# Crocodoctopus/zkstark

Measured on AMD Instinct MI355X. Metric: field-elements/s through LDE+Merkle+FRI (full STARK-101 prover), higher is better.
Workload: dtype u32 (mod 3*2^30+1) + SHA-256

## Files before the change

### zkstark_amd/csrc/kernels.hip

```cpp
#include "kernels.hpp"

#include <cstdlib>

#include "field.hpp"
#include "fieldhash_f64.hpp"
#include "sha256_quad.hpp"
#include "sha256.hpp"

namespace zk {

__device__ __forceinline__ uint32_t pow_lookup(const PowTable& t, uint32_t e) {
    return mont_mul(t.hi[e >> t.lo_bits], t.lo[e & ((1u << t.lo_bits) - 1u)]);
}

constexpr uint32_t R2_MONT = R2;

__device__ uint32_t mont_inv(uint32_t a) {
    uint32_t r = R1, b = a;
    uint32_t e = P - 2;
#pragma unroll 1
    for (int i = 0; i < 32; ++i) {
        if (e & 1) r = mont_mul(r, b);
        b = mont_mul(b, b);
        e >>= 1;
// ... 316 lines not shown
            f2[k] = B == 1 ? fw[k + 2] : fw[k + 4];
            inv2[k] = B == 1 ? iw[k + 2] : iw[k + 4];
            zz[k] = B == 1 ? a.zz[0] : a.zz[k & 1];
        }
    }
    uint32_t x = mont_mul(pow_lookup(a.htab, (uint32_t)i), a.w_mont);
    const uint32_t h = pow_lookup(a.htab, 1u);
    uint32_t r[4];
#pragma unroll
    for (int k = 0; k < 4; ++k) {
        r[k] = compose_eval<false>(a, f0[k], f1[k], f2[k], inv0[k], inv2[k], x, zz[k], a.first, a.last, a.alpha0_mont, a.alpha1g2_mont, 0u);
        if (k < 3) x = mont_mul(x, h);
    }
    reinterpret_cast<uint4*>(a.cp)[i >> 2] = make_uint4(r[0], r[1], r[2], r[3]);
}

hipError_t launch_compose(const ComposeArgs& a, hipStream_t s, Profiler* prof) {
    size_t N = (size_t)1 << a.logN;
    ScopedKernelTimer tm(prof, K_COMPOSE, 8.0 * (double)N, s);
    const bool aligned = ((reinterpret_cast<uintptr_t>(a.f) | reinterpret_cast<uintptr_t>(a.inv_xm1) | reinterpret_cast<uintptr_t>(a.cp)) & 15u) == 0;
    if (a.logN >= 4 && aligned) {
        uint32_t blocks = (uint32_t)((N / 4 + 255) / 256);
        hipLaunchKernelGGL(compose_kernel4, dim3(blocks), dim3(256), 0, s, a);
    } else {
        uint32_t blocks = (uint32_t)((N + 255) / 256);
        hipLaunchKernelGGL(compose_kernel, dim3(blocks), dim3(256), 0, s, a);
    }
    return hipGetLastError();
}

struct FoldRaw { uint32_t u, v, x_hi, x_lo; };
__device__ __forceinline__ FoldRaw fold_fetch(const FoldArgs& a, size_t i) {
    const size_t half = (size_t)1 << (a.log_m - 1);
    const uint32_t e = (uint32_t)(i << a.round);
    FoldRaw r;
    r.u = a.in[i]; r.v = a.in[i + half];
    r.x_hi = a.hinv.hi[e >> a.hinv.lo_bits]; r.x_lo = a.hinv.lo[e & ((1u << a.hinv.lo_bits) - 1u)];
    return r;
}
__device__ __forceinline__ uint32_t fold_finish(const FoldArgs& a, const FoldRaw& r) {
    uint32_t xinv = mont_mul(r.x_hi, r.x_lo);
    uint32_t s = mont_mul(add(r.u, r.v), a.inv2_mont);
    uint32_t d = mont_mul(mont_mul(sub(r.u, r.v), xinv), a.c_mont);
    return add(s, d);
}
__device__ __forceinline__ uint32_t fold_at(const FoldArgs& a, size_t i) { return fold_finish(a, fold_fetch(a, i)); }

__global__ __launch_bounds__(256) void fri_fold_kernel(FoldArgs a) {
    size_t i = (size_t)blockIdx.x * blockDim.x + threadIdx.x;
    if (i >= ((size_t)1 << (a.log_m - 1))) return;
    a.out[i] = fold_at(a, i);
}

__global__ __launch_bounds__(256) void fri_fold_kernel4(FoldArgs a) {
    const size_t half = (size_t)1 << (a.log_m - 1);
    const size_t i = ((size_t)blockIdx.x * blockDim.x + threadIdx.x) * 4;
    if (i >= half) return;
    const uint4 u = reinterpret_cast<const uint4*>(a.in)[i >> 2], v = reinterpret_cast<const uint4*>(a.in)[(i + half) >> 2];
    const uint32_t uu[4] = {u.x, u.y, u.z, u.w}, vv[4] = {v.x, v.y, v.z, v.w};
    uint32_t xinv = pow_lookup(a.hinv, (uint32_t)(i << a.round));
    const uint32_t step = pow_lookup(a.hinv, 1u << a.round);
    uint32_t r[4];
#pragma unroll
    for (int k = 0; k < 4; ++k) {
        const uint32_t sm = mont_mul(add(uu[k], vv[k]), a.inv2_mont);
        const uint32_t d = mont_mul(mont_mul(sub(uu[k], vv[k]), xinv), a.c_mont);
        r[k] = add(sm, d);
        if (k < 3) xinv = mont_mul(xinv, step);
    }
    reinterpret_cast<uint4*>(a.out)[i >> 2] = make_uint4(r[0], r[1], r[2], r[3]);
}

hipError_t launch_fri_fold(const FoldArgs& a, hipStream_t s, Profiler* prof) {
    size_t half = (size_t)1 << (a.log_m - 1);
    ScopedKernelTimer tm(prof, K_FOLD, 12.0 * (double)half, s);
    const bool aligned = ((reinterpret_cast<uintptr_t>(a.in) | reinterpret_cast<uintptr_t>(a.out)) & 15u) == 0;
    if (half >= 4 && aligned) {
        uint32_t blocks = (uint32_t)((half / 4 + 255) / 256);
        hipLaunchKernelGGL(fri_fold_kernel4, dim3(blocks), dim3(256), 0, s, a);
    } else {
        uint32_t blocks = (uint32_t)((half + 255) / 256);
        hipLaunchKernelGGL(fri_fold_kernel, dim3(blocks), dim3(256), 0, s, a);
    }
    return hipGetLastError();
}


__constant__ FieldHashConsts g_fh_consts;
__constant__ FieldHashConsts64 g_fh_consts64;

template <int HASH> struct Hasher;
template <> struct Hasher<0> {
    static __device__ __forceinline__ Digest leaf(uint32_t v) { return sha256_leaf(v); }
    static __device__ __forceinline__ Digest inner(const Digest& l, const Digest& r) { return sha256_inner(l, r); }
};
template <> struct Hasher<1> {
    static __device__ __forceinline__ Digest leaf(uint32_t v) { return fieldhash_leaf64(v, g_fh_consts64); }
    static __device__ __forceinline__ Digest inner(const Digest& l, const Digest& r) { return fieldhash_inner64(l, r, g_fh_consts64); }
};

struct PlainSrc {
    const uint32_t* vals;
    using Raw = uint32_t;
    __device__ __forceinline__ Raw fetch(size_t pos) const { return vals[pos]; }
    __device__ __forceinline__ uint32_t finish(const Raw& r, size_t) const { return r; }
    __device__ __forceinline__ uint32_t load(size_t pos) const { return vals[pos]; }
};
struct FoldSrc {
    FoldArgs a;
    using Raw = FoldRaw;
    __device__ __forceinline__ void prepare() { if (a.dyn) a.c_mont = *a.dyn; }
    __device__ __forceinline__ Raw fetch(size_t pos) const { return fold_fetch(a, pos); }
    __device__ __forceinline__ uint32_t finish(const Raw& r, size_t pos) const { uint32_t v = fold_finish(a, r); a.out[pos] = v; return v; }
    __device__ __forceinline__ uint32_t load(size_t pos) const { return finish(fetch(pos), pos); }
};
struct ComposeSrc {
    ComposeArgs a;
    using Raw = size_t;
    __device__ __forceinline__ Raw fetch(size_t pos) const { return pos; }
    __device__ __forceinline__ uint32_t finish(const Raw& r, size_t) const { return load(r); }
    __device__ __forceinline__ uint32_t load(size_t pos) const { uint32_t v = compose_at(a, pos); a.cp[pos] = v; return v; }
};

struct ComposeBlockSrc {
    ComposeBlockArgs b;
    using Raw = size_t;
    __device__ __forceinline__ uint32_t f_at(size_t t) const {
        const uint32_t gmask = (1u << b.lg) - 1u;
        if (t >> b.log_m) {
            const size_t v = t - ((size_t)1 << b.log_m);
            return b.halo[(v & gmask) * b.halo_stride + (v >> b.lg)];
        }
        const uint32_t log_cl = b.lg + b.log_cnt;
        const size_t piece = ((t >> log_cl) << b.lg) | (t & gmask);
        return b.a.f[(piece << b.log_cnt) | ((t & (((size_t)1 << log_cl) - 1)) >> b.lg)];
    }
    __device__ __forceinline__ Raw fetch(size_t pos) const { return pos; }
    __device__ __forceinline__ uint32_t finish(const Raw& r, size_t) const { return load(r); }
    __device__ __forceinline__ uint32_t load(size_t pos) const {
        const ComposeArgs& a = b.a;
        const size_t B = (size_t)1 << a.log_b;
        const uint32_t f0 = f_at(pos), f1 = f_at(pos + B), f2 = f_at(pos + 2 * B);
        const uint32_t x = mont_mul(pow_lookup(a.htab, b.e0 + (uint32_t)pos), a.w_mont);
        return compose_eval<false>(a, f0, f1, f2, a.inv_xm1[pos], a.inv_xm1[pos + 2 * B], x, a.zz[pos & (B - 1)], a.first, a.last, a.alpha0_mont,
                                   a.alpha1g2_mont, 0u);
    }
};

struct ComposeBatchSrc {
    ComposeArgs a;
    const BatchChal* chal;
    using Raw = size_t;
    __device__ __forceinline__ Raw fetch(size_t pos) const { return pos; }
    __device__ __forceinline__ uint32_t finish(const Raw& r, size_t) const { return load(r); }
    __device__ __forceinline__ uint32_t load(size_t pos) const {
        const size_t b = pos >> a.logN, i = pos & (((size_t)1 << a.logN) - 1);
        const BatchChal c = chal[b];
        uint32_t v = compose_core<true>(a, a.f + (b << a.logN), c.first, c.last, c.alpha0_mont, c.alpha1g2_mont, c.alpha2_mont, i);
        a.cp[pos] = v;
        return v;
    }
};
struct FoldBatchSrc {
    FoldArgs a;
    const BatchChal* chal;
    using Raw = size_t;
    __device__ __forceinline__ Raw fetch(size_t pos) const { return pos; }
    __device__ __forceinline__ uint32_t finish(const Raw& r, size_t) const { return load(r); }
    __device__ __forceinline__ uint32_t load(size_t pos) const {
        const uint32_t lh = a.log_m - 1;
        const size_t half = (size_t)1 << lh, b = pos >> lh, i = pos & (half - 1);
        const uint32_t* in = a.in + (b << a.log_m);
        uint32_t u = in[i], v = in[i + half];
        uint32_t xinv = pow_lookup(a.hinv, (uint32_t)(i << a.round));
        uint32_t s = mont_mul(add(u, v), a.inv2_mont);
        uint32_t d = mont_mul(mont_mul(sub(u, v), xinv), chal[b].c_mont);
        uint32_t r = add(s, d);
        a.out[pos] = r;
        return r;
    }
};

struct InterleaveSrc {
    const uint32_t* recv;
    uint32_t log_parts, log_cnt;
    using Raw = uint32_t;
    __device__ __forceinline__ uint32_t load(size_t pos) const {
        return recv[((pos & (((size_t)1 << log_parts) - 1)) << log_cnt) | (pos >> log_parts)];
    }
    __device__ __forceinline__ Raw fetch(size_t pos) const { return load(pos); }
    __device__ __forceinline__ uint32_t finish(const Raw& r, size_t) const { return r; }
};

template <class S> __device__ __forceinline__ auto src_prepare(S& s, int) -> decltype(s.prepare(), void()) { s.prepare(); }
template <class S> __device__ __forceinline__ void src_prepare(S&, long) {}

constexpr int kMerkleThreads = 256;
constexpr uint32_t kMerkleMaxK = 4;

__device__ __forceinline__ void store_digest(uint32_t* nodes, size_t node, const Digest& d) {
    uint4* q = reinterpret_cast<uint4*>(nodes + node * 8);
    q[0] = make_uint4(d.w[0], d.w[1], d.w[2], d.w[3]);
    q[1] = make_uint4(d.w[4], d.w[5], d.w[6], d.w[7]);
}
__device__ __forceinline__ Digest load_digest(const uint32_t* nodes, size_t node) {
    const uint4* q = reinterpret_cast<const uint4*>(nodes + node * 8);
    uint4 lo = q[0], hi = q[1];
    Digest d;
    d.w[0] = lo.x; d.w[1] = lo.y; d.w[2] = lo.z; d.w[3] = lo.w;
    d.w[4] = hi.x; d.w[5] = hi.y; d.w[6] = hi.z; d.w[7] = hi.w;
    return d;
}

__device__ __forceinline__ Digest lds_digest(const uint4* p) {
    uint4 lo = p[0], hi = p[1];
    Digest d;
    d.w[0] = lo.x; d.w[1] = lo.y; d.w[2] = lo.z; d.w[3] = lo.w;
    d.w[4] = hi.x; d.w[5] = hi.y; d.w[6] = hi.z; d.w[7] = hi.w;
    return d;
}

template <class SRC, bool LEAF, int HASH>
__global__ __launch_bounds__(kMerkleThreads) void merkle_subtree_kernel(SRC src, uint32_t* nodes,
                                                                        uint32_t depth_in, uint32_t k, size_t off) {
    extern __shared__ __attribute__((aligned(16))) uint4 stage[];
    src_prepare(src, 0);
    const uint32_t lane = threadIdx.x & 63u, wave = threadIdx.x >> 6;
    const size_t gwave = (size_t)blockIdx.x * (kMerkleThreads / 64) + wave;
    const size_t base = (gwave << (6 + k)) + off;
    const size_t in_base = ((size_t)1 << depth_in) - 1;
    uint4* my = stage + (size_t)wave * (k + 1) * 128;
    uint4* scratch = my + (size_t)k * 128;
    typename SRC::Raw raw;
    Digest dnext;
    uint32_t val = 0;
    if (LEAF) val = src.load(base + lane - off);
    else dnext = load_digest(nodes, in_base + base + lane);
#pragma unroll 1
    for (uint32_t i = 0; i < (1u << k); ++i) {
        Digest d;
        const size_t pos = base + (size_t)i * 64 + lane;
        const bool more = i + 1 < (1u << k);
        if (LEAF) {
            if (more) raw = src.fetch(pos + 64 - off);
            d = Hasher<HASH>::leaf(val);
            store_digest(nodes, in_base + pos, d);
        } else {
            d = dnext;
            if (more) dnext = load_digest(nodes, in_base + pos + 64);
        }
        uint32_t idx = i, lvl = 0;
#pragma unroll 1
        while (lvl < k) {
            uint4* left = my + lvl * 128;
            uint4* grp = (idx & 1u) ? scratch : left;
            grp[2 * lane] = make_uint4(d.w[0], d.w[1], d.w[2], d.w[3]);
            grp[2 * lane + 1] = make_uint4(d.w[4], d.w[5], d.w[6], d.w[7]);
            if (!(idx & 1u)) break;
            __builtin_amdgcn_fence(__ATOMIC_RELEASE, "wavefront");
            __builtin_amdgcn_wave_barrier();
            const uint4* x = (lane < 32u ? left : scratch - 128) + 4 * lane;
            Digest l = lds_digest(x), r = lds_digest(x + 2);
            __builtin_amdgcn_wave_barrier();
            d = Hasher<HASH>::inner(l, r);
            idx >>= 1;
            ++lvl;
            store_digest(nodes, (((size_t)1 << (depth_in - lvl)) - 1) + (base >> lvl) + (size_t)idx * 64 + lane, d);
        }
        if (LEAF && more) val = src.finish(raw, pos + 64 - off);
    }
}

constexpr int kWgThreads = 256;
#ifndef ZK_FIELD_ROW_MAX_NODES
#define ZK_FIELD_ROW_MAX_NODES 16
#endif
constexpr uint32_t kFieldRowMaxNodes = ZK_FIELD_ROW_MAX_NODES;
static_assert(kFieldRowMaxNodes >= 16 && kFieldRowMaxNodes <= 64, "the row form takes at most four passes of 16 nodes");
#ifndef ZK_FIELD_QUAD_MAX_NODES
#define ZK_FIELD_QUAD_MAX_NODES 64
#endif
constexpr uint32_t kFieldQuadMaxNodes = ZK_FIELD_QUAD_MAX_NODES;
static_assert(kFieldQuadMaxNodes <= 128, "the quad form takes at most two passes of 64 nodes");
#ifndef ZK_FIELD_ROW_LEAF_MAX
#define ZK_FIELD_ROW_LEAF_MAX 32
#endif
constexpr uint32_t kFieldRowLeafMax = ZK_FIELD_ROW_LEAF_MAX;
static_assert(kFieldRowLeafMax <= 64, "the row form takes at most four passes of 16 leaves");
constexpr uint32_t kWgMaxLog = 10;

__device__ __forceinline__ void lds_store(uint4* p, const Digest& d) {
    p[0] = make_uint4(d.w[0], d.w[1], d.w[2], d.w[3]);
    p[1] = make_uint4(d.w[4], d.w[5], d.w[6], d.w[7]);
}

#ifndef ZK_WG_RELAXED_PUBLISH
#define ZK_WG_RELAXED_PUBLISH 1
#endif
constexpr bool kWgRelaxedPublish = ZK_WG_RELAXED_PUBLISH != 0;
__device__ __forceinline__ void publish_node(uint32_t* nodes, size_t node, const uint4* lvl0, uint32_t tid) {
    if (tid < 8) __hip_atomic_store(nodes + node * 8 + tid, reinterpret_cast<const uint32_t*>(lvl0)[tid], __ATOMIC_RELAXED, __HIP_MEMORY_SCOPE_AGENT);
    asm volatile("s_waitcnt vmcnt(0)" ::: "memory");
}
__device__ __forceinline__ Digest load_digest_agent(const uint32_t* nodes, size_t node) {
    const unsigned long long* q = reinterpret_cast<const unsigned long long*>(nodes + node * 8);
    Digest d;
#pragma unroll
    for (int i = 0; i < 4; ++i) {
        const unsigned long long v = __hip_atomic_load(q + i, __ATOMIC_RELAXED, __HIP_MEMORY_SCOPE_AGENT);
        d.w[2 * i] = (uint32_t)v; d.w[2 * i + 1] = (uint32_t)(v >> 32);
    }
    return d;
}

#ifdef ZK_WG_TRACE
constexpr uint32_t kWgTraceSlots = 48, kWgTraceLaunches = 8192;
__device__ unsigned long long g_wg_trace[kWgTraceLaunches][kWgTraceSlots];
__device__ unsigned int g_wg_trace_n, g_wg_trace_cur;
#define WG_STAMP(slot) do { if (threadIdx.x == 0 && wg_rec < kWgTraceLaunches && (slot) < kWgTraceSlots) g_wg_trace[wg_rec][(slot)] = __builtin_amdgcn_s_memrealtime(); } while (0)
#else
#define WG_STAMP(slot) do { } while (0)
#endif

template <class SRC, bool LEAF, int HASH>
__global__ __launch_bounds__(kWgThreads) void merkle_wg_kernel(SRC src, uint32_t* nodes, uint32_t depth_in, uint32_t j,
                                                               MailArgs mail, size_t off, uint32_t j2, uint32_t lds_log) {
    extern __shared__ __attribute__((aligned(16))) uint4 lvl[];
    src_prepare(src, 0);
    uint32_t* xch = reinterpret_cast<uint32_t*>(lvl + ((size_t)2 << lds_log));
    const uint32_t tid = threadIdx.x;
    uint32_t cnt = 1u << j;
    size_t first = ((size_t)blockIdx.x << j) + off;
    uint32_t d_in = depth_in, lv = j;
    const size_t in_base = ((size_t)1 << depth_in) - 1;
    QuadLane ql;
    if (HASH == 0) ql = quad_lane(tid);
#ifdef ZK_WG_TRACE
    uint32_t wg_rec = 0xffffffffu;
    if (blockIdx.x == 0 && tid == 0) {
        wg_rec = atomicAdd(&g_wg_trace_n, 1u);
        __hip_atomic_store(&g_wg_trace_cur, wg_rec, __ATOMIC_RELAXED, __HIP_MEMORY_SCOPE_AGENT);
        if (wg_rec < kWgTraceLaunches) {
            for (uint32_t i = 0; i < kWgTraceSlots; ++i) g_wg_trace[wg_rec][i] = 0;
            g_wg_trace[wg_rec][0] = (unsigned long long)depth_in | ((unsigned long long)j << 8) | ((unsigned long long)j2 << 16) | ((unsigned long long)(LEAF ? 1 : 0) << 24) |
                                    ((unsigned long long)HASH << 25) | ((unsigned long long)(mail.mailbox ? mail.top + 1 : 0) << 26) | ((unsigned long long)gridDim.x << 32);
        }
    }
    WG_STAMP(1);
#endif
    constexpr uint32_t kPer = (1u << kWgMaxLog) / kWgThreads;
    if (LEAF && HASH == 1 && cnt <= kFieldRowLeafMax) {
        const uint32_t g = tid & 15u, grp = tid >> 4;
#pragma unroll 1
        for (uint32_t b = 0; b * 16 < cnt; ++b) {
            const uint32_t i = b * 16 + grp;
            const uint32_t ii = i < cnt ? i : 0u;
            const uint32_t v = src.finish(src.fetch(first + ii - off), first + ii - off);
            const uint32_t word = g == 0 ? v : g == 15 ? 1u : 0u;
            const uint32_t res = fieldhash_inner_row16_f64(word, g, g_fh_consts64);
            if (i < cnt && g < 8) {
                nodes[(in_base + first + i) * 8 + g] = res;
                reinterpret_cast<uint32_t*>(&lvl[2 * i])[g] = res;
            }
        }
    } else if (LEAF) {
        typename SRC::Raw raw[kPer] = {};
#pragma unroll
        for (uint32_t u = 0; u < kPer; ++u)
            if (tid + u * kWgThreads < cnt) raw[u] = src.fetch(first + tid + u * kWgThreads - off);
#pragma unroll 1
        for (uint32_t i = tid; i < cnt; i += kWgThreads) {
            const Digest d = Hasher<HASH>::leaf(src.finish(raw[0], first + i - off));
            store_digest(nodes, in_base + first + i, d);
            lds_store(&lvl[2 * i], d);
#pragma unroll
            for (uint32_t u = 0; u + 1 < kPer; ++u) raw[u] = raw[u + 1];
        }
    } else {
        Digest dd[kPer];
#pragma unroll
        for (uint32_t u = 0; u < kPer; ++u)
            if (tid + u * kWgThreads < cnt) dd[u] = load_digest(nodes, in_base + first + tid + u * kWgThreads);
#pragma unroll
        for (uint32_t u = 0; u < kPer; ++u)
            if (tid + u * kWgThreads < cnt) lds_store(&lvl[2 * (tid + u * kWgThreads)], dd[u]);
    }
    if (LEAF && mail.dump_src) __threadfence();
    __syncthreads();
    WG_STAMP(2);
#pragma unroll 1
  for (uint32_t phase = 0;; ++phase) {
#pragma unroll 1
    for (uint32_t t = 1; t <= lv; ++t) {
        const uint32_t w = cnt >> t;
        const size_t out_base = (((size_t)1 << (d_in - t)) - 1) + (first >> t);
        WG_STAMP((phase ? 24u : 2u) + t - 1u);
        if (HASH == 0 && w <= 64) {
            const uint32_t lane = tid & 63u, wave = tid >> 6;
            const uint32_t node = wave * 16 + (lane >> 4) * 4 + (lane & 3u), role = (lane >> 2) & 3u;
            const bool busy = wave * 16 < w;
            uint32_t o[4];
            if (busy) sha256_inner_quad(reinterpret_cast<const uint32_t*>(&lvl[4 * (node < w ? node : 0u)]), ql, o);
            __syncthreads();
            if (busy && node < w && role < 2) {
                const uint4 v = make_uint4(o[0], o[1], o[2], o[3]);
                lvl[2 * node + (role ^ 1u)] = v;
                reinterpret_cast<uint4*>(nodes + (out_base + node) * 8)[role ^ 1u] = v;
            }
            __syncthreads();
            continue;
        }
        if (HASH == 0 && w <= 128) {
            const bool is_main = tid < 128;
            const uint32_t node = tid & 127u;
            const bool active = node < w;
            uint32_t wv[16];
            uint32_t st[8];
            if (active) {
                Digest l = lds_digest(&lvl[4 * node]), r = lds_digest(&lvl[4 * node + 2]);
#pragma unroll
                for (int i = 0; i < 8; ++i) { wv[i] = l.w[i]; wv[8 + i] = r.w[i]; st[i] = SHA_IV[i]; }
            }
            uint32_t* xb0 = xch;
            uint32_t* xb1 = xch + 16 * 128;
            if (active) {
                if (is_main) sha256_rounds16<0>(st, wv);
                else { sha256_schedule16(wv);
#pragma unroll
                       for (int i = 0; i < 16; ++i) xb0[i * 128 + node] = wv[i]; }
            }
            __syncthreads();
            if (active) {
                if (is_main) {
#pragma unroll
                    for (int i = 0; i < 16; ++i) wv[i] = xb0[i * 128 + node];
                    sha256_rounds16<16>(st, wv);
                } else { sha256_schedule16(wv);
#pragma unroll
                         for (int i = 0; i < 16; ++i) xb1[i * 128 + node] = wv[i]; }
            }
            __syncthreads();
            if (active) {
                if (is_main) {
#pragma unroll
                    for (int i = 0; i < 16; ++i) wv[i] = xb1[i * 128 + node];
                    sha256_rounds16<32>(st, wv);
                } else { sha256_schedule16(wv);
#pragma unroll
                         for (int i = 0; i < 16; ++i) xb0[i * 128 + node] = wv[i]; }
            }
            __syncthreads();
            Digest d0;
            if (active && is_main) {
#pragma unroll
                for (int i = 0; i < 16; ++i) wv[i] = xb0[i * 128 + node];
                sha256_rounds16<48>(st, wv);
#pragma unroll
                for (int i = 0; i < 8; ++i) d0.w[i] = st[i] + SHA_IV[i];
                uint32_t pad[16] = {0x80000000u, 0, 0, 0, 0, 0, 0, 0, 0, 0, 0, 0, 0, 0, 0, 512u};
                sha256_compress(d0.w, pad);
            }
            __syncthreads();
            if (active && is_main) { lds_store(&lvl[2 * node], d0); store_digest(nodes, out_base + node, d0); }
            __syncthreads();
            continue;
        }
        if (HASH == 1 && w > kFieldRowMaxNodes && w <= kFieldQuadMaxNodes) {
            const uint32_t q = tid & 3u, grp = tid >> 2;
            uint32_t res[2][4];
#pragma unroll
            for (uint32_t b = 0; b < 2; ++b) {
                if (b * 64 >= w) break;
                const uint32_t node = b * 64 + grp;
                const uint4 v = lvl[4 * (node < w ? node : 0u) + q];
                const uint32_t in[4] = {v.x, v.y, v.z, v.w};
                fieldhash_inner_quad_f64(in, q, res[b], g_fh_consts64);
            }
            __syncthreads();
#pragma unroll
            for (uint32_t b = 0; b < 2; ++b) {
                if (b * 64 >= w) break;
                const uint32_t node = b * 64 + grp;
                if (node < w && q < 2) {
                    const uint4 o = make_uint4(res[b][0], res[b][1], res[b][2], res[b][3]);
                    lvl[2 * node + q] = o;
                    reinterpret_cast<uint4*>(nodes + (out_base + node) * 8)[q] = o;
                }
            }
            __syncthreads();
            continue;
        }
        if (HASH == 1 && w <= kFieldRowMaxNodes) {
            const uint32_t g = tid & 15u, grp = tid >> 4;
            uint32_t res[4];
#pragma unroll
            for (uint32_t b = 0; b < 4; ++b) {
                if (b * 16 >= w) break;
                const uint32_t node = b * 16 + grp;
                const uint32_t* words = reinterpret_cast<const uint32_t*>(&lvl[4 * (node < w ? node : 0u)]);
                res[b] = fieldhash_inner_row16_f64(words[g], g, g_fh_consts64);
            }
            __syncthreads();
#pragma unroll
            for (uint32_t b = 0; b < 4; ++b) {
                if (b * 16 >= w) break;
                const uint32_t node = b * 16 + grp;
                if (node < w && g < 8) {
                    reinterpret_cast<uint32_t*>(&lvl[2 * node])[g] = res[b];
                    nodes[(out_base + node) * 8 + g] = res[b];
                }
            }
            __syncthreads();
            continue;
        }
        Digest d0, d1;
        const bool a0 = tid < w, a1 = tid + kWgThreads < w;
        if (a0) d0 = Hasher<HASH>::inner(lds_digest(&lvl[4 * tid]), lds_digest(&lvl[4 * tid + 2]));
        if (a1) d1 = Hasher<HASH>::inner(lds_digest(&lvl[4 * (tid + kWgThreads)]), lds_digest(&lvl[4 * (tid + kWgThreads) + 2]));
        __syncthreads();
        if (a0) { lds_store(&lvl[2 * tid], d0); store_digest(nodes, out_base + tid, d0); }
        if (a1) { lds_store(&lvl[2 * (tid + kWgThreads)], d1); store_digest(nodes, out_base + tid + kWgThreads, d1); }
        __syncthreads();
    }
    WG_STAMP((phase ? 24u : 2u) + lv);
    if (phase == 1 || j2 == 0) break;
    __shared__ uint32_t go_on;
    if (gridDim.x > 1) {
        if (kWgRelaxedPublish) {
            publish_node(nodes, (((size_t)1 << (depth_in - j)) - 1) + blockIdx.x, lvl, tid);
        } else {
            asm volatile("s_waitcnt vmcnt(0)" ::: "memory");
            __syncthreads();
        }
    }
    if (tid == 0) {
        uint32_t last = 1;
        if (gridDim.x > 1) {
            last = (kWgRelaxedPublish ? __hip_atomic_fetch_add(mail.counter + 1, 1u, __ATOMIC_RELAXED, __HIP_MEMORY_SCOPE_AGENT)
                                      : __hip_atomic_fetch_add(mail.counter + 1, 1u, __ATOMIC_ACQ_REL, __HIP_MEMORY_SCOPE_AGENT)) == gridDim.x - 1;
            if (last) __hip_atomic_store(mail.counter + 1, 0u, __ATOMIC_RELAXED, __HIP_MEMORY_SCOPE_AGENT);
        }
        go_on = last;
    }
    __syncthreads();
    if (!go_on) return;
    if (kWgRelaxedPublish && LEAF && mail.dump_src) __builtin_amdgcn_fence(__ATOMIC_ACQUIRE, "agent");
#ifdef ZK_WG_TRACE
    if (tid == 0) wg_rec = __hip_atomic_load(&g_wg_trace_cur, __ATOMIC_RELAXED, __HIP_MEMORY_SCOPE_AGENT);
    WG_STAMP(15);
#endif
    d_in = depth_in - j; lv = j2; cnt = gridDim.x; first = 0;
    {
        const size_t base2 = ((size_t)1 << d_in) - 1;
        Digest dd[kPer];
#pragma unroll
        for (uint32_t u = 0; u < kPer; ++u)
            if (tid + u * kWgThreads < cnt)
                dd[u] = (kWgRelaxedPublish && gridDim.x > 1) ? load_digest_agent(nodes, base2 + tid + u * kWgThreads) : load_digest(nodes, base2 + tid + u * kWgThreads);
#pragma unroll
        for (uint32_t u = 0; u < kPer; ++u)
            if (tid + u * kWgThreads < cnt) lds_store(&lvl[2 * (tid + u * kWgThreads)], dd[u]);
    }
    __syncthreads();
    WG_STAMP(16);
  }
    if (mail.mailbox && depth_in - j - j2 == mail.top && off == 0) {
        __shared__ uint32_t is_last;
        const bool relaxed = kWgRelaxedPublish && gridDim.x > 1 && j2 == 0 && mail.dump_src == nullptr;
        if (relaxed) publish_node(nodes, (((size_t)1 << mail.top) - 1) + blockIdx.x, lvl, tid);
        if (tid == 0) {
            uint32_t last = 1;
            if (gridDim.x > 1 && j2 == 0) {
                last = (relaxed ? __hip_atomic_fetch_add(mail.counter, 1u, __ATOMIC_RELAXED, __HIP_MEMORY_SCOPE_AGENT)
                                : __hip_atomic_fetch_add(mail.counter, 1u, __ATOMIC_ACQ_REL, __HIP_MEMORY_SCOPE_AGENT)) == gridDim.x - 1;
                if (last) __hip_atomic_store(mail.counter, 0u, __ATOMIC_RELAXED, __HIP_MEMORY_SCOPE_AGENT);
            }
            is_last = last;
        }
        __syncthreads();
        if (is_last) {
#ifdef ZK_WG_TRACE
            if (tid == 0 && wg_rec == 0xffffffffu) wg_rec = __hip_atomic_load(&g_wg_trace_cur, __ATOMIC_RELAXED, __HIP_MEMORY_SCOPE_AGENT);
            WG_STAMP(40);
#endif
            const uint4* sq = reinterpret_cast<const uint4*>(nodes + (((size_t)1 << mail.top) - 1) * 8);
            uint4* dq = reinterpret_cast<uint4*>(mail.mailbox + kMailDigests);
            if (relaxed) {
                for (uint32_t i = tid; i < (1u << mail.top); i += kWgThreads) {
                    const Digest d = load_digest_agent(nodes, (((size_t)1 << mail.top) - 1) + i);
                    dq[2 * i] = make_uint4(d.w[0], d.w[1], d.w[2], d.w[3]);
                    dq[2 * i + 1] = make_uint4(d.w[4], d.w[5], d.w[6], d.w[7]);
                }
            } else {
                for (uint32_t i = tid; i < (2u << mail.top); i += kWgThreads) dq[i] = sq[i];
            }
            if (mail.dump_src) {
                const uint4* sv = reinterpret_cast<const uint4*>(mail.dump_src);
                uint4* dv = reinterpret_cast<uint4*>(mail.mailbox + mail.vals_off);
                for (uint32_t i = tid; i < (1u << mail.dump_log) / 4; i += kWgThreads) dv[i] = sv[i];
            }
            __threadfence_system();
            __syncthreads();
            WG_STAMP(41);
            if (tid == 0) __hip_atomic_store(&mail.mailbox[0], mail.seq, __ATOMIC_RELEASE, __HIP_MEMORY_SCOPE_SYSTEM);
            WG_STAMP(42);
        }
    }
}

#ifdef ZK_WG_TRACE
void dump_wg_trace() {
    const char* path = getenv("ZK_WG_TRACE_FILE");
    unsigned int n = 0;
    if (!path || hipMemcpyFromSymbol(&n, HIP_SYMBOL(g_wg_trace_n), sizeof n) != hipSuccess || !n) return;
    if (n > kWgTraceLaunches) n = kWgTraceLaunches;
    std::vector<unsigned long long> rec((size_t)n * kWgTraceSlots);
    if (hipMemcpyFromSymbol(rec.data(), HIP_SYMBOL(g_wg_trace), rec.size() * 8) != hipSuccess) return;
    FILE* f = fopen(path, "a");
    if (!f) return;
    for (unsigned int r = 0; r < n; ++r) {
        const unsigned long long* x = &rec[(size_t)r * kWgTraceSlots];
        const unsigned long long m = x[0];
        fprintf(f, "wg depth_in=%llu j=%llu j2=%llu leaf=%llu hash=%llu top=%lld wgs=%llu abs0=%llu :", m & 255, (m >> 8) & 255, (m >> 16) & 255, (m >> 24) & 1, (m >> 25) & 1,
                (long long)((m >> 26) & 63) - 1, m >> 32, x[1]);
        for (uint32_t i = 1; i < kWgTraceSlots; ++i) fprintf(f, " %lld", x[i] ? (long long)(x[i] - x[1]) : -1LL);
        fprintf(f, "\n");
    }
    fclose(f);
    const unsigned int zero = 0;
    (void)hipMemcpyToSymbol(HIP_SYMBOL(g_wg_trace_n), &zero, sizeof zero);
}
#endif

static double merkle_bytes(bool leaf, uint32_t depth, uint32_t k) {
    double in = (double)((size_t)1 << depth);
    double produced = (leaf ? in : 0.0) + in * (1.0 - 1.0 / (double)((size_t)1 << k));
    return (leaf ? 4.0 : 32.0) * in + 32.0 * produced;
}
static double merkle_ops(bool leaf, uint32_t depth, uint32_t k, int hash) {
    double in = (double)((size_t)1 << depth);
    double lo = hash ? kFieldLeafOps : kShaLeafOps, io = hash ? kFieldInnerOps : kShaInnerOps;
    return (leaf ? in * lo : 0.0) + in * (1.0 - 1.0 / (double)((size_t)1 << k)) * io;
}

static hipError_t ensure_fieldhash_consts() {
    static bool done[64] = {false};
    int dev = 0;
    hipError_t e = hipGetDevice(&dev);
    if (e != hipSuccess) return e;
    if (dev < 0 || dev >= 64 || done[dev]) return hipSuccess;
    FieldHashConsts c;
    fieldhash_make_consts(c);
    e = hipMemcpyToSymbol(HIP_SYMBOL(g_fh_consts), &c, sizeof c);
    if (e != hipSuccess) return e;
    static FieldHashConsts64 c64;
    fieldhash_make_consts64(c, c64);
    e = hipMemcpyToSymbol(HIP_SYMBOL(g_fh_consts64), &c64, sizeof c64);
    if (e == hipSuccess) done[dev] = true;
    return e;
}

#ifndef ZK_MERKLE_MAX_K
#define ZK_MERKLE_MAX_K 4
#endif
#ifndef ZK_MERKLE_LATENCY_LOG
#define ZK_MERKLE_LATENCY_LOG 17
#endif
#ifndef ZK_MERKLE_CHUNK_K
#define ZK_MERKLE_CHUNK_K 3
#endif
static_assert(ZK_MERKLE_MAX_K >= 1 && ZK_MERKLE_MAX_K <= (int)kMerkleMaxK && ZK_MERKLE_CHUNK_K >= 1 && ZK_MERKLE_CHUNK_K <= (int)kMerkleMaxK, "levels per launch");
static_assert(ZK_MERKLE_LATENCY_LOG >= 12 && ZK_MERKLE_LATENCY_LOG <= 24, "latency switch");
static uint32_t g_merkle_latency_log = ZK_MERKLE_LATENCY_LOG;
static constexpr uint32_t merkle_max_k() { return ZK_MERKLE_MAX_K; }
static uint32_t merkle_latency_log() { return __atomic_load_n(&g_merkle_latency_log, __ATOMIC_RELAXED); }
bool set_merkle_latency_log(uint32_t v) {
    if (v == 0) v = ZK_MERKLE_LATENCY_LOG;
    if (v < 12 || v > 24) return false;
    __atomic_store_n(&g_merkle_latency_log, v, __ATOMIC_RELAXED);
    return true;
}

static double wg_level_us(uint32_t w, int hash) {
    if (w == 0) return 0.0;
    if (hash) return w <= kFieldRowMaxNodes ? (double)((w + 15) / 16) * 3.7 : w <= kFieldQuadMaxNodes ? (double)((w + 63) / 64) * 5.3 : (double)((w + 255) / 256) * 10.8;
    return w <= 64 ? 3.1 : w <= 128 ? 4.9 : (double)((w + 255) / 256) * 4.6;
}
static double wg_phase_us(bool leaf, uint32_t cnt_log, uint32_t levels, int hash, uint32_t blocks) {
    const uint32_t cnt = 1u << cnt_log;
    double us = !leaf ? 1.0
                : hash ? (cnt <= kFieldRowLeafMax ? (double)((cnt + 15) / 16) * 3.7 : (double)((cnt + 255) / 256) * 10.8)
                       : (double)((cnt + 255) / 256) * 2.6;
    for (uint32_t t = 1; t <= levels; ++t) us += wg_level_us(cnt >> t, hash);
    return blocks > 256 ? us * (double)blocks / 256.0 : us;
}
#ifndef ZK_MERKLE_CONTINUATION
#define ZK_MERKLE_CONTINUATION 1
#endif
static constexpr bool g_merkle_continuation = ZK_MERKLE_CONTINUATION != 0;
constexpr double kContinueUs = 6.0;
constexpr double kLaunchUs = 10.0;

template <class SRC>
static hipError_t merkle_build_t(SRC src, double src_bytes, uint32_t log_m, uint32_t* nodes, hipStream_t s, Profiler* prof,
                                 const MailArgs& mail_in, int hash, uint32_t log_sub = 0xffffffffu, size_t chunk = 0,
                                 bool leaf_mode = true, uint32_t tp_floor = 0) {
    if (hash) {
        hipError_t e = ensure_fieldhash_consts();
        if (e != hipSuccess) return e;
    }
    if (log_sub == 0xffffffffu) log_sub = log_m;
    const uint32_t stop = log_m - log_sub;
    uint32_t depth = log_m;
    bool leaf = leaf_mode;
    const PlainSrc none{nullptr};
    auto first_bytes = [&](double b) { return leaf ? b - 4.0 * (double)((size_t)1 << log_sub) + src_bytes : b; };
    const uint32_t kMerkleLatencyLog = merkle_latency_log();
    auto off_at = [&](uint32_t d) { return (size_t)chunk << (d - stop); };
    const bool throughput_only = tp_floor != 0;
    const uint32_t floor_depth = throughput_only ? tp_floor : stop + kMerkleLatencyLog;
    while (depth > floor_depth) {
        uint32_t k = depth - floor_depth;
        if (k > merkle_max_k()) k = merkle_max_k();
        size_t lanes = (size_t)1 << (depth - stop - k);
        uint32_t blocks = (uint32_t)(lanes / kMerkleThreads);
        size_t sh = (size_t)(kMerkleThreads / 64) * (k + 1) * 128 * sizeof(uint4);
        ScopedKernelTimer tm(prof, leaf ? K_MERKLE_LEAF : K_MERKLE_INNER, first_bytes(merkle_bytes(leaf, depth - stop, k)), s, merkle_ops(leaf, depth - stop, k, hash));
        if (hash) {
            if (leaf) hipLaunchKernelGGL((merkle_subtree_kernel<SRC, true, 1>), dim3(blocks), dim3(kMerkleThreads), sh, s, src, nodes, depth, k, off_at(depth));
            else hipLaunchKernelGGL((merkle_subtree_kernel<PlainSrc, false, 1>), dim3(blocks), dim3(kMerkleThreads), sh, s, none, nodes, depth, k, off_at(depth));
        } else {
            if (leaf) hipLaunchKernelGGL((merkle_subtree_kernel<SRC, true, 0>), dim3(blocks), dim3(kMerkleThreads), sh, s, src, nodes, depth, k, off_at(depth));
            else hipLaunchKernelGGL((merkle_subtree_kernel<PlainSrc, false, 0>), dim3(blocks), dim3(kMerkleThreads), sh, s, none, nodes, depth, k, off_at(depth));
        }
        leaf = false;
        depth -= k;
    }
    if (throughput_only) return hipGetLastError();
    MailArgs mail = mail_in;
    if (stop != 0 || mail.top >= log_m) mail.top = 0;
    const uint32_t end = stop == 0 ? mail.top : stop;
    auto launch_wg = [&](uint32_t j, uint32_t j2) {
        const uint32_t span = depth - stop;
        const uint32_t blocks = 1u << (span - j);
        const uint32_t lds_log = j2 && span - j > j ? span - j : j;
        const size_t sh = ((size_t)2 << lds_log) * sizeof(uint4) + 2 * 16 * 128 * sizeof(uint32_t);
        ScopedKernelTimer tm(prof, K_MERKLE_TOP, first_bytes(merkle_bytes(leaf, span, j)) + (j2 ? merkle_bytes(false, span - j, j2) : 0.0), s,
                             merkle_ops(leaf, span, j, hash) + (j2 ? merkle_ops(false, span - j, j2, hash) : 0.0));
        if (hash) {
            if (leaf) hipLaunchKernelGGL((merkle_wg_kernel<SRC, true, 1>), dim3(blocks), dim3(kWgThreads), sh, s, src, nodes, depth, j, mail, off_at(depth), j2, lds_log);
            else hipLaunchKernelGGL((merkle_wg_kernel<PlainSrc, false, 1>), dim3(blocks), dim3(kWgThreads), sh, s, none, nodes, depth, j, mail, off_at(depth), j2, lds_log);
        } else {
            if (leaf) hipLaunchKernelGGL((merkle_wg_kernel<SRC, true, 0>), dim3(blocks), dim3(kWgThreads), sh, s, src, nodes, depth, j, mail, off_at(depth), j2, lds_log);
            else hipLaunchKernelGGL((merkle_wg_kernel<PlainSrc, false, 0>), dim3(blocks), dim3(kWgThreads), sh, s, none, nodes, depth, j, mail, off_at(depth), j2, lds_log);
        }
        leaf = false;
        depth -= j + j2;
    };
    const bool may_continue = stop == 0 && mail.counter != nullptr && g_merkle_continuation;
    do {
        const uint32_t span = depth - stop;
        const uint32_t levels = depth - end;
        const uint32_t launches = levels ? (levels + kWgMaxLog - 1) / kWgMaxLog : 1;
        const uint32_t jn = (levels + launches - 1) / launches;
        uint32_t best_j = jn, best_j2 = 0;
        if (may_continue && levels <= 2 * kWgMaxLog) {
            double best = wg_phase_us(leaf, jn, jn, hash, 1u << (span - jn));
            if (launches == 2 && span - jn <= kWgMaxLog) best += kLaunchUs + wg_phase_us(false, span - jn, levels - jn, hash, 1);
            else if (launches > 1) best = 0.0;
            for (uint32_t j = 1; j < levels && j <= kWgMaxLog; ++j) {
                const uint32_t j2 = levels - j;
                if (j2 > kWgMaxLog || span - j > kWgMaxLog) continue;
                const double us = wg_phase_us(leaf, j, j, hash, 1u << (span - j)) + kContinueUs + wg_phase_us(false, span - j, j2, hash, 1);
                if (us < best) { best = us; best_j = j; best_j2 = j2; }
            }
        }
        launch_wg(best_j, best_j2);
    } while (depth > end);
    return hipGetLastError();
}

hipError_t launch_merkle_build(const uint32_t* vals, uint32_t log_m, uint32_t* nodes, hipStream_t s, Profiler* prof,
                               const MailArgs& mail, int hash) {
    return merkle_build_t(PlainSrc{vals}, 4.0 * (double)((size_t)1 << log_m), log_m, nodes, s, prof, mail, hash);
}
hipError_t launch_merkle_build_interleaved(const uint32_t* recv, uint32_t log_parts, uint32_t log_cnt, uint32_t* nodes, hipStream_t s,
                                           Profiler* prof, int hash, const MailArgs& mail) {
    uint32_t log_m = log_parts + log_cnt;
    return merkle_build_t(InterleaveSrc{recv, log_parts, log_cnt}, 4.0 * (double)((size_t)1 << log_m), log_m, nodes, s, prof, mail, hash);
}
static constexpr uint32_t merkle_chunk_k() { return ZK_MERKLE_CHUNK_K; }
static uint32_t chunk_handover_depth(uint32_t log_m, uint32_t log_chunks) {
    const uint32_t lat = merkle_latency_log();
    if (!(log_m > lat && lat >= log_chunks + 8)) return log_chunks;
    uint32_t k = log_m - lat < merkle_max_k() ? log_m - lat : merkle_max_k();
    if (k > merkle_chunk_k()) k = merkle_chunk_k();
    return log_m - k;
}
uint32_t merkle_finish_start_depth(uint32_t log_m, uint32_t log_chunks) { return chunk_handover_depth(log_m, log_chunks); }
hipError_t launch_merkle_build_chunk(const uint32_t* recv, uint32_t log_parts, uint32_t log_cnt, uint32_t* nodes, uint32_t log_m,
                                     uint32_t chunk, hipStream_t s, Profiler* prof, int hash) {
    uint32_t log_sub = log_parts + log_cnt;
    const uint32_t h = chunk_handover_depth(log_m, log_m - log_sub);
    return merkle_build_t(InterleaveSrc{recv, log_parts, log_cnt}, 4.0 * (double)((size_t)1 << log_sub), log_m, nodes, s, prof, MailArgs{}, hash,
                          log_sub, chunk, true, h != log_m - log_sub ? h : 0u);
}
hipError_t launch_merkle_finish(uint32_t* nodes, uint32_t log_m, uint32_t log_chunks, hipStream_t s, Profiler* prof, int hash,
                                const MailArgs& mail) {
    const uint32_t start = chunk_handover_depth(log_m, log_chunks);
    if (start == 0) return hipSuccess;
    return merkle_build_t(PlainSrc{nullptr}, 0.0, start, nodes, s, prof, mail, hash, start, 0, false);
}
hipError_t launch_fold_merkle(const FoldArgs& a, uint32_t* nodes, hipStream_t s, Profiler* prof, const MailArgs& mail, int hash) {
    uint32_t log_out = a.log_m - 1;
    return merkle_build_t(FoldSrc{a}, 12.0 * (double)((size_t)1 << log_out), log_out, nodes, s, prof, mail, hash);
}
hipError_t launch_compose_merkle(const ComposeArgs& a, uint32_t* nodes, hipStream_t s, Profiler* prof, const MailArgs& mail, int hash) {
    return merkle_build_t(ComposeSrc{a}, 8.0 * (double)((size_t)1 << a.logN), a.logN, nodes, s, prof, mail, hash);
}

hipError_t launch_compose_block_merkle(const ComposeBlockArgs& b, uint32_t* nodes, hipStream_t s, Profiler* prof, const MailArgs& mail, int hash) {
    return merkle_build_t(ComposeBlockSrc{b}, 8.0 * (double)((size_t)1 << b.log_m), b.log_m, nodes, s, prof, mail, hash);
}

hipError_t launch_compose_merkle_batch(const ComposeBatchArgs& a, uint32_t log_batch, uint32_t* nodes, hipStream_t s, Profiler* prof,
                                       const MailArgs& mail, int hash) {
    uint32_t log_m = a.a.logN + log_batch;
    return merkle_build_t(ComposeBatchSrc{a.a, a.chal}, 8.0 * (double)((size_t)1 << log_m), log_m, nodes, s, prof, mail, hash);
}
hipError_t launch_fold_merkle_batch(const FoldBatchArgs& a, uint32_t log_batch, uint32_t* nodes, hipStream_t s, Profiler* prof,
                                    const MailArgs& mail, int hash) {
    uint32_t log_out = a.a.log_m - 1 + log_batch;
    return merkle_build_t(FoldBatchSrc{a.a, a.chal}, 12.0 * (double)((size_t)1 << log_out), log_out, nodes, s, prof, mail, hash);
}

__global__ __launch_bounds__(1024) void scatter_kernel(const uint32_t* stage, const ScatterSeg* segs, uint32_t* trees, uint32_t* layers) {
    const ScatterSeg sg = segs[blockIdx.x];
    uint32_t* dst = (sg.kind ? layers : trees) + sg.dst;
    const uint32_t* src = stage + sg.src;
    if (((sg.src | sg.dst | sg.words) & 3) == 0) {
        const uint4* s4 = reinterpret_cast<const uint4*>(src);
        uint4* d4 = reinterpret_cast<uint4*>(dst);
        for (uint32_t i = threadIdx.x; i < sg.words / 4; i += blockDim.x) d4[i] = s4[i];
    } else {
        for (uint32_t i = threadIdx.x; i < sg.words; i += blockDim.x) dst[i] = src[i];
    }
}
hipError_t launch_scatter(const uint32_t* stage, const ScatterSeg* segs, uint32_t count, double words, uint32_t* trees, uint32_t* layers,
                          hipStream_t s, Profiler* prof) {
    if (!count) return hipSuccess;
    ScopedKernelTimer tm(prof, K_GATHER, 8.0 * words, s);
    hipLaunchKernelGGL(scatter_kernel, dim3(count), dim3(1024), 0, s, stage, segs, trees, layers);
    return hipGetLastError();
}

template <int HASH>
__global__ __launch_bounds__(256) void hash_chain_probe_kernel(uint32_t* out, uint32_t seed, uint32_t hashes, unsigned long long* rec) {
    Digest d;
#pragma unroll
    for (int i = 0; i < 8; ++i) d.w[i] = (seed * (uint32_t)(i + 1) + threadIdx.x + blockIdx.x * 977u) % P;
    const unsigned long long c0 = __builtin_amdgcn_s_memtime(), r0 = __builtin_amdgcn_s_memrealtime();
#pragma unroll 1
    for (uint32_t it = 0; it < hashes; ++it) {
        Digest r = d;
        r.w[0] ^= seed;
        if (HASH) r.w[0] &= 0x7fffffffu;
        d = Hasher<HASH>::inner(d, r);
    }
    const unsigned long long c1 = __builtin_amdgcn_s_memtime(), r1 = __builtin_amdgcn_s_memrealtime();
    uint32_t x = 0;
#pragma unroll
    for (int i = 0; i < 8; ++i) x ^= d.w[i];
    out[blockIdx.x * 256 + threadIdx.x] = x;
    if (rec && (threadIdx.x & 63) == 0) {
        rec[((size_t)blockIdx.x * 4 + (threadIdx.x >> 6)) * 2] = c1 - c0;
        rec[((size_t)blockIdx.x * 4 + (threadIdx.x >> 6)) * 2 + 1] = r1 - r0;
    }
}
hipError_t launch_hash_chain_probe(int hash, uint32_t blocks, uint32_t* out, uint32_t seed, uint32_t hashes, unsigned long long* rec, hipStream_t s) {
    if (hash) {
        hipError_t e = ensure_fieldhash_consts();
        if (e != hipSuccess) return e;
        hipLaunchKernelGGL(hash_chain_probe_kernel<1>, dim3(blocks), dim3(256), 0, s, out, seed, hashes, rec);
    } else {
        hipLaunchKernelGGL(hash_chain_probe_kernel<0>, dim3(blocks), dim3(256), 0, s, out, seed, hashes, rec);
    }
    return hipGetLastError();
}

__global__ __launch_bounds__(256) void fieldhash_forms_kernel(uint32_t seed, uint32_t* bad, uint32_t* first_bad) {
    const uint32_t t = blockIdx.x * blockDim.x + threadIdx.x;
    uint32_t x = (t + 1u) * 2654435761u + seed;
    auto rnd = [&]() { x ^= x << 13; x ^= x >> 17; x ^= x << 5; return x; };
    Digest l, r;
#pragma unroll
    for (int i = 0; i < 8; ++i) { l.w[i] = rnd() % P; r.w[i] = rnd() % P; }
    if ((t & 15u) == 1) { l.w[t & 7u] = 0; r.w[(t >> 4) & 7u] = P - 1; }
    if ((t & 15u) == 2) {
#pragma unroll
        for (int i = 0; i < 8; ++i) { l.w[i] = P - 1; r.w[i] = P - 1; }
    }
    if ((t & 15u) == 3) { l.w[0] = 0xFFFFFFFFu; r.w[7] = P; r.w[3] = P + 5; }
    if ((t & 15u) == 4) {
#pragma unroll
        for (int i = 0; i < 8; ++i) { l.w[i] = 0; r.w[i] = 0; }
    }
    uint32_t v = rnd();
    if ((t & 7u) == 0) v = (t & 8u) ? 0xFFFFFFFFu : P - 1;
    if (t == 5) v = 0;
// ... 213 lines not shown
```

Measured before the change: 2.938 billion.

## Spread mailbox posting across workgroups instead of serial last-block copy

Each workgroup now writes its own top-level digest, plus its slice of the dumped values, straight into the host-visible mailbox using system-scope relaxed atomic stores. The last workgroup then only bumps the sequence word with a release store. Before, the last workgroup copied every top digest and the whole value dump by itself after the counter handoff, and paid for an acquire fence and a system-wide threadfence. This moves that serial tail work off the critical path. It relies on relaxed system-scope stores being visible before the release store of the sequence word. That ordering across workgroups is subtle and could let the host read stale data.

```diff
diff --git a/zkstark_amd/csrc/kernels.hip b/zkstark_amd/csrc/kernels.hip
--- a/zkstark_amd/csrc/kernels.hip
+++ b/zkstark_amd/csrc/kernels.hip
@@ -642,6 +642,17 @@
     if (tid < 8) __hip_atomic_store(nodes + node * 8 + tid, reinterpret_cast<const uint32_t*>(lvl0)[tid], __ATOMIC_RELAXED, __HIP_MEMORY_SCOPE_AGENT);
     asm volatile("s_waitcnt vmcnt(0)" ::: "memory");
 }
+__device__ __forceinline__ void post_words(uint32_t* dst, const uint32_t* src, uint32_t words, uint32_t tid) {
+    const unsigned long long* s = reinterpret_cast<const unsigned long long*>(src);
+    unsigned long long* d = reinterpret_cast<unsigned long long*>(dst);
+    for (uint32_t k = tid; k < words / 2; k += kWgThreads) __hip_atomic_store(d + k, s[k], __ATOMIC_RELAXED, __HIP_MEMORY_SCOPE_SYSTEM);
+}
+__device__ __forceinline__ void post_words_grid(uint32_t* dst, const uint32_t* src, uint32_t words, uint32_t tid) {
+    const unsigned long long* s = reinterpret_cast<const unsigned long long*>(src);
+    unsigned long long* d = reinterpret_cast<unsigned long long*>(dst);
+    for (uint32_t k = blockIdx.x * kWgThreads + tid; k < words / 2; k += gridDim.x * kWgThreads)
+        __hip_atomic_store(d + k, s[k], __ATOMIC_RELAXED, __HIP_MEMORY_SCOPE_SYSTEM);
+}
 __device__ __forceinline__ Digest load_digest_agent(const uint32_t* nodes, size_t node) {
     const unsigned long long* q = reinterpret_cast<const unsigned long long*>(nodes + node * 8);
     Digest d;
@@ -725,7 +736,13 @@
         for (uint32_t u = 0; u < kPer; ++u)
             if (tid + u * kWgThreads < cnt) lds_store(&lvl[2 * (tid + u * kWgThreads)], dd[u]);
     }
-    if (LEAF && mail.dump_src) __threadfence();
+    const bool posts = mail.mailbox && depth_in - j - j2 == mail.top && off == 0;
+    if (posts && mail.dump_src) {
+        __syncthreads();
+        if (LEAF) post_words(mail.mailbox + mail.vals_off + first, mail.dump_src + first, cnt, tid);
+        else post_words_grid(mail.mailbox + mail.vals_off, mail.dump_src, 1u << mail.dump_log, tid);
+        if (j2) asm volatile("s_waitcnt vmcnt(0)" ::: "memory");
+    }
     __syncthreads();
     WG_STAMP(2);
 #pragma unroll 1
@@ -884,7 +901,6 @@
     }
     __syncthreads();
     if (!go_on) return;
-    if (kWgRelaxedPublish && LEAF && mail.dump_src) __builtin_amdgcn_fence(__ATOMIC_ACQUIRE, "agent");
 #ifdef ZK_WG_TRACE
     if (tid == 0) wg_rec = __hip_atomic_load(&g_wg_trace_cur, __ATOMIC_RELAXED, __HIP_MEMORY_SCOPE_AGENT);
     WG_STAMP(15);
@@ -904,47 +920,36 @@
     __syncthreads();
     WG_STAMP(16);
   }
-    if (mail.mailbox && depth_in - j - j2 == mail.top && off == 0) {
+    if (posts) {
+#ifdef ZK_WG_TRACE
+        const unsigned long long t40 = __builtin_amdgcn_s_memrealtime();
+#endif
         __shared__ uint32_t is_last;
-        const bool relaxed = kWgRelaxedPublish && gridDim.x > 1 && j2 == 0 && mail.dump_src == nullptr;
-        if (relaxed) publish_node(nodes, (((size_t)1 << mail.top) - 1) + blockIdx.x, lvl, tid);
+        const bool spread = gridDim.x > 1 && j2 == 0;
+        if (spread) post_words(mail.mailbox + kMailDigests + 8 * blockIdx.x, reinterpret_cast<const uint32_t*>(lvl), 8, tid);
+        else post_words(mail.mailbox + kMailDigests, reinterpret_cast<const uint32_t*>(lvl), 8u << mail.top, tid);
+        asm volatile("s_waitcnt vmcnt(0)" ::: "memory");
+        __syncthreads();
+#ifdef ZK_WG_TRACE
+        const unsigned long long t41 = __builtin_amdgcn_s_memrealtime();
+#endif
         if (tid == 0) {
             uint32_t last = 1;
-            if (gridDim.x > 1 && j2 == 0) {
-                last = (relaxed ? __hip_atomic_fetch_add(mail.counter, 1u, __ATOMIC_RELAXED, __HIP_MEMORY_SCOPE_AGENT)
-                                : __hip_atomic_fetch_add(mail.counter, 1u, __ATOMIC_ACQ_REL, __HIP_MEMORY_SCOPE_AGENT)) == gridDim.x - 1;
+            if (spread) {
+                last = __hip_atomic_fetch_add(mail.counter, 1u, __ATOMIC_RELAXED, __HIP_MEMORY_SCOPE_AGENT) == gridDim.x - 1;
                 if (last) __hip_atomic_store(mail.counter, 0u, __ATOMIC_RELAXED, __HIP_MEMORY_SCOPE_AGENT);
             }
             is_last = last;
+            if (last) {
+#ifdef ZK_WG_TRACE
+                if (wg_rec == 0xffffffffu) wg_rec = __hip_atomic_load(&g_wg_trace_cur, __ATOMIC_RELAXED, __HIP_MEMORY_SCOPE_AGENT);
+                if (wg_rec < kWgTraceLaunches) { g_wg_trace[wg_rec][40] = t40; g_wg_trace[wg_rec][41] = t41; }
+#endif
+                __hip_atomic_store(&mail.mailbox[0], mail.seq, __ATOMIC_RELEASE, __HIP_MEMORY_SCOPE_SYSTEM);
+            }
         }
         __syncthreads();
-        if (is_last) {
-#ifdef ZK_WG_TRACE
-            if (tid == 0 && wg_rec == 0xffffffffu) wg_rec = __hip_atomic_load(&g_wg_trace_cur, __ATOMIC_RELAXED, __HIP_MEMORY_SCOPE_AGENT);
-            WG_STAMP(40);
-#endif
-            const uint4* sq = reinterpret_cast<const uint4*>(nodes + (((size_t)1 << mail.top) - 1) * 8);
-            uint4* dq = reinterpret_cast<uint4*>(mail.mailbox + kMailDigests);
-            if (relaxed) {
-                for (uint32_t i = tid; i < (1u << mail.top); i += kWgThreads) {
-                    const Digest d = load_digest_agent(nodes, (((size_t)1 << mail.top) - 1) + i);
-                    dq[2 * i] = make_uint4(d.w[0], d.w[1], d.w[2], d.w[3]);
-                    dq[2 * i + 1] = make_uint4(d.w[4], d.w[5], d.w[6], d.w[7]);
-                }
-            } else {
-                for (uint32_t i = tid; i < (2u << mail.top); i += kWgThreads) dq[i] = sq[i];
-            }
-            if (mail.dump_src) {
-                const uint4* sv = reinterpret_cast<const uint4*>(mail.dump_src);
-                uint4* dv = reinterpret_cast<uint4*>(mail.mailbox + mail.vals_off);
-                for (uint32_t i = tid; i < (1u << mail.dump_log) / 4; i += kWgThreads) dv[i] = sv[i];
-            }
-            __threadfence_system();
-            __syncthreads();
-            WG_STAMP(41);
-            if (tid == 0) __hip_atomic_store(&mail.mailbox[0], mail.seq, __ATOMIC_RELEASE, __HIP_MEMORY_SCOPE_SYSTEM);
-            WG_STAMP(42);
-        }
+        if (is_last) WG_STAMP(42);
     }
 }
 
```

Result: no change. 2.960 billion, median of 6 (+0.8%).
